# mpotse/ParMmg

Hardware: AMD Instinct MI355X
Metric: new-mesh points located+interpolated/sec (Mpts/s) and HBM GB/s, 1/2/4/8 GPU (higher is better)
Workload: dtype f64

## Files before the change

parmmg_amd/csrc/pmmg_hip.hip:

```cpp
#include <hip/hip_ext.h>
#include <hip/hip_runtime.h>

#include <math.h>
#include <stdarg.h>
#include <stdint.h>
#include <stdio.h>
#include <stdlib.h>
#include <string.h>

#include <algorithm>
#include <chrono>
#include <condition_variable>
#include <functional>
#include <mutex>
#include <string>
#include <thread>
#include <type_traits>
#include <vector>

#include "pmmg_device.hpp"
#include "pmmg_prep.hpp"
#include "pmmg_sort.hpp"
#include "pmmg_vol.hpp"
#include "pmmg_bdy.hpp"
#include "pmmg_fallback.hpp"
#include "pmmg_snapshot.hpp"
#include "pmmg_quality.hpp"
#include "pmmg_meshstats.hpp"
#include "pmmg_graph.hpp"
#include "pmmg_comm.hpp"

using namespace pmmg;

namespace {


typedef void (*VolFn)(Bg, const Frame *, const unsigned long long *, int, const double *, const uint8_t *,
                      const int *, int, DevStats *, Slots, int *, int8_t *, int, const int *, int, ContArgs, MapArgs);

struct LayoutEntry {
  int c[6];
  VolFn fn;
  VolFn fn_packed;
  VolFn fn_packed2;
  VolFn map_fn, map_fn_packed, map_fn_packed2;
};

template <int NP, int A, int B, int C, int D, int E, int F, int MAP = 0>
constexpr VolFn packed_fn() {
  using L = PackedLayout<A, B, C, D, E, F>;
  if constexpr (L::valid() && L::passes_ok(NP)) return k_vol<NP, A, B, C, D, E, F, MAP>;
  else return nullptr;
}
#define PMMG_LAYOUT(a, b, c, d, e, f)                                                                    \
  {{a, b, c, d, e, f}, k_vol<0, a, b, c, d, e, f>, packed_fn<1, a, b, c, d, e, f>(),                    \
   packed_fn<2, a, b, c, d, e, f>(), k_vol<0, a, b, c, d, e, f, 1>, packed_fn<1, a, b, c, d, e, f, 1>(), \
   packed_fn<2, a, b, c, d, e, f, 1>()}
const LayoutEntry kLayouts[] = {
    PMMG_LAYOUT(6, 1, 3, 6, 0, 0), PMMG_LAYOUT(6, 1, 3, 6, 1, 0), PMMG_LAYOUT(1, 1, 0, 0, 0, 0),
    PMMG_LAYOUT(1, 1, 1, 1, 1, 1), PMMG_LAYOUT(1, 1, 1, 0, 0, 0), PMMG_LAYOUT(6, 0, 0, 0, 0, 0),
    PMMG_LAYOUT(1, 0, 0, 0, 0, 0), PMMG_LAYOUT(6, 1, 0, 0, 0, 0), PMMG_LAYOUT(1, 1, 3, 6, 0, 0),
    PMMG_LAYOUT(0, 0, 0, 0, 0, 0),
};
#undef PMMG_LAYOUT

VolFn pick_layout(const Slots &S, int passes = 0, bool map = false) {
  for (const LayoutEntry &e : kLayouts) {
    int n = 0;
    while (n < 6 && e.c[n] > 0) n++;
    if (n != S.n) continue;
    bool ok = true;
    for (int j = 0; j < n; j++) ok = ok && (S.s[j].code == e.c[j]);
    if (!ok) continue;
    if (!S.rec) return map ? e.map_fn : e.fn;
    if (passes == 0) {
      int k = 0;
      for (int j = 0; j < n; j++) k += e.c[j];
      passes = k > 8 ? 2 : 1;
    }
    const VolFn p1 = map ? e.map_fn_packed : e.fn_packed, p2 = map ? e.map_fn_packed2 : e.fn_packed2;
    const VolFn a = passes == 2 ? p2 : p1, b = passes == 2 ? p1 : p2;
    return a ? a : b;
  }
  if (S.rec) return nullptr;
  return map ? k_vol<0, -1, 0, 0, 0, 0, 0, 1> : k_vol<0, -1, 0, 0, 0, 0, 0>;
}

bool packed_supported(int met_size, int nfield, const int *fsize) {
  Slots S{};
  S.rec = reinterpret_cast<const double *>(16);
  if (met_size) S.s[S.n++].code = met_size;
  for (int j = 0; j < nfield && S.n < kMaxSlot; j++) S.s[S.n++].code = fsize[j];
  return pick_layout(S) != nullptr;
}

}


struct CtxBufs {
  DevBuf o_xyz, o_tetv, o_adja, o_triv, o_adjt, o_met, o_rec;
  std::vector<DevBuf> o_f;
  DevBuf o_tet4;
  DevBuf frame, stats, grid, sgrid, order_v, order_b, xq;
  DevBuf cohd;
  DevBuf axh;
  DevBuf bkeys, bkeys2, bvals, bvals2;
  DevBuf rs_hist, rs_csum;
  DevBuf cls_cnt;
  DevBuf oflag;
  DevBuf qmin;
  DevBuf fb_vol, fb_bdy, best, nac, cres, bbest, bnac, bcres;
  DevBuf fbp_vol, fbp_bdy;
  DevBuf fbg_vol_c, fbg_vol_u, fbg_vol_i, fbg_bdy_c, fbg_bdy_u, fbg_bdy_i;
  DevBuf h_xyz, h_cls, h_met, h_elem, h_hit;
  std::vector<DevBuf> h_f;
  SnapCache snap_cache;
  StatsCache stats_cache;
  GraphCache graph_cache;
  struct Kept {
    DevBuf xyz, met;
    std::vector<DevBuf> f;
    int np = 0, met_size = 0;
    std::vector<int> fsize;
    bool valid = false;
  };
  std::vector<Kept> kept;
  DevBuf carry_dsrc, carry_need, carry_ids, carry_cnt, carry_rows, carry_bc;
  DevBuf map_own;
  DevBuf map_need;
  DevBuf start_tab;
  DevBuf ag_send, ag_recv, ag_off, ag_chk;
};

enum {
  EV_START, EV_FRAME, EV_PREP, EV_ORDER, EV_VOL0, EV_WALK, EV_JOIN, EV_END, EV_BDY0, EV_BDY1, EV_RESET,
  EV_SB0, EV_ORDER2, EV_FILL, EV_COUNT
};

struct pmmg_hip_ctx : CtxBufs {
  int device = 0;
  int options = 0;
  hipStream_t stream = nullptr;
  hipStream_t stream2 = nullptr;
  hipStream_t stream3 = nullptr;
  hipStream_t stream_f = nullptr;
  char err[512] = {0};
  Bg bg{};
  int met_size = 0;
  int nfield = 0;
  std::vector<int> fsize;
  std::vector<const double *> fin;
  const double *met = nullptr;
  const double *rec = nullptr;
  int rstride = 0;
  void *grid_clean_p = nullptr, *sgrid_clean_p = nullptr;
  long long grid_clean_n = 0, sgrid_clean_n = 0;
  hipEvent_t ev[EV_COUNT] = {};
  bool pending = false;
  void *stage[2] = {nullptr, nullptr};
  void *stage_dev[2] = {nullptr, nullptr};
  hipEvent_t stage_ev[2] = {};
  int stage_i = 0;
  struct Pool *pool = nullptr;
  int edge_hash = 1;
  hipStream_t cstream = nullptr;
  std::thread snap;
  int snap_ok = 1;
  int verbose = 0;
  int tpc = 8;
  int pack_passes = 0;
  int ev_vol0 = EV_VOL0;
  int *flag_host = nullptr;
  int *flag_host_dev = nullptr;
  int srf_g = 0;
  int srf_mult = 8;
  int bin_bits = kBinBitsCoherent;
  int maxstep = 1024;
  int fanmax = kFanMax;
  int last_host_np = 0, last_host_met = 0;
  std::vector<int> last_host_fsize;
  int carry_slot = -1, carry_np = 0;
  bool carry_bg = false;
  std::vector<int> carry_src;
  int64_t bytes_up = 0;
  const int *map_src = nullptr;
  int map_np = 0;
  bool start_valid = false;
  std::vector<pmmg_hip_ctx *> lanes;
  bool borrowed_streams = false;
  ncclComm_t comm = nullptr;
  bool comm_owned = false;
  int comm_rank = 0, comm_size = 0;
  int group_lanes = 3;
  struct Pool *lane_pool = nullptr;
  int filter_steps = 64;
};

static void set_err(pmmg_hip_ctx *c, const char *fmt, ...) {
  if (!c) return;
  va_list ap;
  va_start(ap, fmt);
  vsnprintf(c->err, sizeof(c->err), fmt, ap);
  va_end(ap);
  fprintf(stderr, "[parmmg_hip] %s\n", c->err);
}

#define HIPCK(ctx, expr)                                                                             \
  do {                                                                                               \
    hipError_t e_ = (expr);                                                                          \
    if (e_ != hipSuccess) {                                                                          \
      set_err((ctx), "%s failed: %s (%s:%d)", #expr, hipGetErrorString(e_), __FILE__, __LINE__);   \
      return 0;                                                                                      \
    }                                                                                                \
  } while (0)

static hipError_t ctx_d2h(pmmg_hip_ctx *c, void *dst, const void *src, size_t n) {
  hipError_t e = hipMemcpyAsync(dst, src, n, hipMemcpyDeviceToHost, c->stream);
  return e != hipSuccess ? e : hipStreamSynchronize(c->stream);
}

static int ensure(pmmg_hip_ctx *c, DevBuf &b, size_t bytes) {
  const hipError_t e = b.ensure(bytes);
  if (e != hipSuccess) {
    set_err(c, "hipMalloc(&b.p, bytes) failed: %s (%s:%d)", hipGetErrorString(e), __FILE__, __LINE__);
    return 0;
  }
  return 1;
}

static int copy_stream(pmmg_hip_ctx *c) {
  if (!c->cstream) HIPCK(c, hipStreamCreateWithFlags(&c->cstream, hipStreamNonBlocking));
  return 1;
}


struct Pool {
  std::vector<std::thread> th;
  std::mutex mu;
  std::condition_variable cv, done;
  std::function<void(size_t, size_t)> fn;
  size_t n = 0, parts = 0, next = 0, left = 0;
  unsigned long long gen = 0;
  bool stop = false;
  explicit Pool(int nthreads) {
    for (int t = 0; t < nthreads; t++) th.emplace_back([this] { loop(); });
  }
  ~Pool() {
    {
      std::lock_guard<std::mutex> g(mu);
      stop = true;
    }
    cv.notify_all();
    for (auto &t : th) t.join();
  }
  bool take(size_t &b, size_t &e) {
    if (next >= parts) return false;
    const size_t p = next++;
    b = n * p / parts;
    e = n * (p + 1) / parts;
    return true;
  }
  void loop() {
    unsigned long long seen = 0;
    std::unique_lock<std::mutex> lk(mu);
    for (;;) {
      cv.wait(lk, [&] { return stop || gen != seen; });
      if (stop) return;
      seen = gen;
      size_t b, e;
      while (take(b, e)) {
        lk.unlock();
        fn(b, e);
        lk.lock();
        if (--left == 0) done.notify_all();
      }
    }
  }
  void run(size_t count, size_t nparts, std::function<void(size_t, size_t)> f) {
    if (nparts <= 1 || th.empty()) {
      f(0, count);
      return;
    }
    std::unique_lock<std::mutex> lk(mu);
    fn = std::move(f);
    n = count;
    parts = nparts;
    next = 0;
    left = nparts;
    gen++;
    cv.notify_all();
    size_t b, e;
    while (take(b, e)) {
      lk.unlock();
      fn(b, e);
      lk.lock();
      left--;
    }
    done.wait(lk, [&] { return left == 0; });
  }
};

static int env_int(const char *name, int def);

constexpr size_t kStageBytes = 32u << 20;
constexpr size_t kStageMin = 4u << 20;
constexpr unsigned long long kSentinel = 0x7FF4A5A5A5A5A5A5ULL;

__global__ __launch_bounds__(kBlock) void k_copy16(const ntd2 *src, ntd2 *dst, long long n) {
  for (long long j = blockIdx.x * (long long)blockDim.x + threadIdx.x; j < n; j += (long long)gridDim.x * blockDim.x)
    __builtin_nontemporal_store(__builtin_nontemporal_load(src + j), dst + j);
}
__global__ __launch_bounds__(kBlock) void k_copy1(const char *src, char *dst, long long n) {
  for (long long j = blockIdx.x * (long long)blockDim.x + threadIdx.x; j < n; j += (long long)gridDim.x * blockDim.x)
    dst[j] = src[j];
}

static int stage_ready(pmmg_hip_ctx *c) {
  if (c->stage[0]) return 1;
  for (int b = 0; b < 2; b++) {
    HIPCK(c, hipHostMalloc(&c->stage[b], kStageBytes, hipHostMallocDefault));
    HIPCK(c, hipHostGetDevicePointer(&c->stage_dev[b], c->stage[b], 0));
    HIPCK(c, hipEventCreateWithFlags(&c->stage_ev[b], hipEventDisableTiming));
  }
  if (!c->pool) {
    const int hw = (int)std::thread::hardware_concurrency();
    c->pool = new Pool(env_int("PMMG_HIP_HOST_THREADS", hw > 16 ? 16 : (hw > 1 ? hw : 1)) - 1);
  }
  return 1;
}

static void par_copy(pmmg_hip_ctx *c, void *dst, const void *src, size_t n) {
  const size_t parts = n >= (8u << 20) ? c->pool->th.size() + 1 : 1;
  c->pool->run(n, parts, [&](size_t b, size_t e) { memcpy((char *)dst + b, (const char *)src + b, e - b); });
}

static int h2d(pmmg_hip_ctx *c, void *dst, const void *src, size_t bytes, hipStream_t s) {
  if (bytes == 0) return 1;
  c->bytes_up += (int64_t)bytes;
  if (bytes < kStageMin) {
    HIPCK(c, hipMemcpyAsync(dst, src, bytes, hipMemcpyHostToDevice, s));
    return 1;
  }
  if (!stage_ready(c)) return 0;
  for (size_t off = 0; off < bytes;) {
    const int b = c->stage_i;
    c->stage_i ^= 1;
    const size_t n = bytes - off < kStageBytes ? bytes - off : kStageBytes;
    HIPCK(c, hipEventSynchronize(c->stage_ev[b]));
    par_copy(c, c->stage[b], (const char *)src + off, n);
    HIPCK(c, hipMemcpyAsync((char *)dst + off, c->stage[b], n, hipMemcpyHostToDevice, s));
    HIPCK(c, hipEventRecord(c->stage_ev[b], s));
    off += n;
  }
  return 1;
}

struct AllRows {
  bool operator()(size_t, const char *) const { return true; }
};
static double now_s() {
  return std::chrono::duration<double>(std::chrono::steady_clock::now().time_since_epoch()).count();
}

template <class Keep>
static int d2h_rows(pmmg_hip_ctx *c, void *dst, const void *src, size_t nrows, size_t row, const Keep &keep) {
  const size_t bytes = nrows * row;
  if (bytes == 0) return 1;
  if (!stage_ready(c)) return 0;
  double t_wait = 0.0;
  const double t_start = now_s();
  const size_t per = kStageBytes / row;
  const size_t nch = (nrows + per - 1) / per;
  auto issue = [&](size_t j) -> int {
    const int b = (int)(j & 1);
    const size_t r0 = j * per, n = (nrows - r0 < per ? nrows - r0 : per) * row;
    const char *from = (const char *)src + r0 * row;
    if (((uintptr_t)from & 15) == 0 && (n & 15) == 0) {
      hipLaunchKernelGGL(k_copy16, dim3(1024), dim3(kBlock), 0, c->stream, (const ntd2 *)from, (ntd2 *)c->stage_dev[b],
                         (long long)(n / 16));
    } else {
      hipLaunchKernelGGL(k_copy1, dim3(1024), dim3(kBlock), 0, c->stream, from, (char *)c->stage_dev[b], (long long)n);
    }
    HIPCK(c, hipGetLastError());
    HIPCK(c, hipEventRecord(c->stage_ev[b], c->stream));
    return 1;
  };
  if (!issue(0)) return 0;
  for (size_t j = 0; j < nch; j++) {
    const int b = (int)(j & 1);
    const double t0 = now_s();
    HIPCK(c, hipEventSynchronize(c->stage_ev[b]));
    const double t1 = now_s();
    t_wait += t1 - t0;
    if (j + 1 < nch && !issue(j + 1)) return 0;
    const size_t r0 = j * per, nr = nrows - r0 < per ? nrows - r0 : per;
    const char *sb = (const char *)c->stage[b];
    char *db = (char *)dst + r0 * row;
    if constexpr (std::is_same<Keep, AllRows>::value) {
      par_copy(c, db, sb, nr * row);
    } else {
      c->pool->run(nr, nr >= 65536 ? c->pool->th.size() + 1 : 1, [&](size_t a, size_t e) {
        size_t r = a;
        while (r < e) {
          while (r < e && !keep(r0 + r, sb + r * row)) r++;
          const size_t s0 = r;
          while (r < e && keep(r0 + r, sb + r * row)) r++;
          if (r > s0) memcpy(db + s0 * row, sb + s0 * row, (r - s0) * row);
        }
      });
    }
  }
  if (c->verbose)
    fprintf(stderr, "[parmmg_hip] d2h %zu rows x %zu B: %.2f ms DMA wait, %.2f ms in total\n", nrows, row,
            1e3 * t_wait, 1e3 * (now_s() - t_start));
  return 1;
}

static int upload(pmmg_hip_ctx *c, DevBuf &b, const void *src, size_t bytes, hipStream_t s = nullptr) {
  if (!ensure(c, b, bytes)) return 0;
  return h2d(c, b.p, src, bytes, s ? s : c->stream);
}

static void invalidate_bg(pmmg_hip_ctx *c) {
  c->bg.ne = c->bg.nt = c->bg.np = 0;
  c->bg.tetv = c->bg.adja = nullptr;
  c->bg.triv = c->bg.adjt = nullptr;
  c->bg.xyz = nullptr;
  c->start_valid = false;
}

static int snap_join(pmmg_hip_ctx *c) {
  if (c->snap.joinable()) c->snap.join();
  if (!c->snap_ok) {
    c->snap_ok = 1;
    invalidate_bg(c);
    return 0;
  }
  return 1;
}
// ... 537 lines not shown
    set_err(c, "set_solutions_packed: a carry-over is armed; it takes pmmg_hip_set_solutions (the kept rows are "
               "per-solution arrays)");
    carry_disarm(c);
    return 0;
  }
  c->met_size = met_size;
  c->nfield = nfield;
  c->fsize.assign(field_size, field_size + nfield);
  c->fin.assign(nfield, nullptr);
  c->met = nullptr;
  c->rstride = (K + 1) & ~1;
  if (where == PMMG_HIP_DEVICE) {
    c->rec = rec;
    return 1;
  }
  if (!copy_stream(c) || !upload(c, c->o_rec, rec, sizeof(double) * c->rstride * np, c->cstream)) return 0;
  c->rec = (const double *)c->o_rec.p;
  HIPCK(c, hipStreamSynchronize(c->cstream));
  return 1;
}

constexpr int kSmallGroup = 1 << 20;

static int grid_dim(long long n, int per_cell, int gmax) {
  double g = cbrt((double)n / (double)per_cell);
  int gi = (int)g;
  if (gi < 1) gi = 1;
  if (gi > gmax) gi = gmax;
  return gi;
}

static int blocks_for(long long n, int cap) {
  long long b = (n + kBlock - 1) / kBlock;
  if (b < 1) b = 1;
  if (b > cap) b = cap;
  return (int)b;
}

static void launch_vol_fallbacks(pmmg_hip_ctx *c, const Slots &S, const double *xyz_new, int *elem_out,
                                 int8_t *hit_out, hipEvent_t stop = nullptr) {
  const Bg &bg = c->bg;
  hipStream_t s = c->stream;
  DevStats *st = (DevStats *)c->stats.p;
  const int *fb = (const int *)c->fb_vol.p;
  const int gv = (int)std::min<long long>(kFbGridVol, std::max<long long>(64, bg.ne / 16384)) & ~7;
  hipLaunchKernelGGL(k_vol_exhaust_accept, dim3(gv), dim3(kBlock), 0, s, bg, xyz_new, fb, st,
                     (int *)c->best.p, (int *)c->nac.p, (const int *)c->fbg_vol_c.p, (const int *)c->fbg_vol_i.p, S,
                     elem_out, hit_out);
  hipExtLaunchKernelGGL(k_vol_exhaust_closest, dim3(gv), dim3(kBlock), 0, s, nullptr, stop, 0, bg, xyz_new, fb, st,
                        (const int *)c->nac.p, (FbPart *)c->fbp_vol.p, (int *)c->cres.p, S, elem_out, hit_out);
}

static void launch_bdy_fallbacks(pmmg_hip_ctx *c, hipStream_t s, const Slots &S, const double *xyz_new,
                                 int *elem_out, int8_t *hit_out, hipEvent_t stop = nullptr) {
  const Bg &bg = c->bg;
  DevStats *st = (DevStats *)c->stats.p;
  const int *fb = (const int *)c->fb_bdy.p;
  const int gb = (int)std::min<long long>(kFbGridBdy, std::max<long long>(32, bg.nt / 4096)) & ~7;
  hipLaunchKernelGGL(k_bdy_exhaust_accept, dim3(gb), dim3(kBlock), 0, s, bg, xyz_new, fb, st,
                     (int *)c->bbest.p, (int *)c->bnac.p, (const int *)c->fbg_bdy_c.p, (const int *)c->fbg_bdy_i.p, S,
                     elem_out, hit_out);
  hipExtLaunchKernelGGL(k_bdy_exhaust_closest, dim3(gb), dim3(kBlock), 0, s, nullptr, stop, 0, bg, xyz_new, fb, st,
                        (const int *)c->bnac.p, (FbPart *)c->fbp_bdy.p, (int *)c->bcres.p, S, elem_out, hit_out);
}

static int start_tables(pmmg_hip_ctx *c) {
  if (c->start_valid) return 1;
  const Bg &bg = c->bg;
  const size_t n = 2 * (size_t)bg.np;
  if (!ensure(c, c->start_tab, sizeof(int) * n)) return 0;
  unsigned *tab = (unsigned *)c->start_tab.p;
  HIPCK(c, hipMemsetAsync(tab, 0xFF, sizeof(int) * n, c->stream));
  hipLaunchKernelGGL(k_start_tet, dim3(blocks_for(bg.ne, 16384)), dim3(kBlock), 0, c->stream, bg, tab);
  if (bg.nt > 0)
    hipLaunchKernelGGL(k_start_tri, dim3(blocks_for(bg.nt, 4096)), dim3(kBlock), 0, c->stream, bg, tab + bg.np);
  hipLaunchKernelGGL(k_start_fin, dim3(blocks_for((long long)n, 4096)), dim3(kBlock), 0, c->stream, tab, (long long)n);
  HIPCK(c, hipGetLastError());
  c->start_valid = true;
  return 1;
}


constexpr int kSeedLanes = 4;
constexpr int kBboxStride = 64;
constexpr int kHistStride = 256;
constexpr int kBdyBpx = 512;
constexpr int kXcdRun = 64;

struct Call {
  pmmg_hip_ctx *c;
  int np_new;
  const double *xyz_new;
  const uint8_t *pclass;
  int *elem_out;
  int8_t *hit_out;
  Bg bg;
  hipStream_t s, sb, sc;
  Slots S;
  VolFn vol_fn;
  MapArgs ma;
  int *need;
  int force;
  int g, gs;
  long long ng, nsg, ncls;
  Frame *fr;
  DevStats *st;
  unsigned long long *grid, *sgrid;
  int *order_v, *order_b;
  const int *flag;
};

static int call_slots(Call &k, double *met_out, double *const *fields_out, double *rec_out, const int *map_src) {
  pmmg_hip_ctx *c = k.c;
  Slots &S = k.S;
  S.n = 0;
  S.has_met = c->met_size ? 1 : 0;
  if (rec_out && !c->rec) {
    set_err(c, "locate_interp_rec: output records need packed input records (pmmg_hip_set_solutions_packed)");
    return 0;
  }
  if (c->met_size) {
    if (!met_out && !rec_out) {
      set_err(c, "locate_interp: met_out is NULL");
      return 0;
    }
    S.s[S.n++] = Slot{c->met, met_out, c->met_size, c->met_size, c->met_size};
  }
  for (int j = 0; j < c->nfield; j++) {
    if (!rec_out && (!fields_out || !fields_out[j])) {
      set_err(c, "locate_interp: fields_out[%d] is NULL", j);
      return 0;
    }
    S.s[S.n++] = Slot{c->fin[j], rec_out ? nullptr : fields_out[j], c->fsize[j], c->fsize[j], c->fsize[j]};
  }
  if (c->rec) {
    S.rec = c->rec;
    int off = 0;
    for (int j = 0; j < S.n; j++) {
      S.s[j].in = c->rec + off;
      S.s[j].istride = c->rstride;
      if (rec_out) {
        S.s[j].out = rec_out + off;
        S.s[j].ostride = c->rstride;
      }
      off += S.s[j].code;
    }
    S.rec_out = rec_out;
  }
  k.vol_fn = pick_layout(S, c->pack_passes, map_src != nullptr);
  if (!k.vol_fn) {
    set_err(c, "locate_interp: no packed-record kernel for this slot layout");
    return 0;
  }
  k.ma = MapArgs{nullptr, nullptr, nullptr};
  k.need = nullptr;
  if (map_src) {
    if (!start_tables(c) || !ensure(c, c->map_need, 2 * sizeof(int))) return 0;
    k.need = (int *)c->map_need.p;
    k.ma = MapArgs{map_src, (const int *)c->start_tab.p, (const int *)c->start_tab.p + k.bg.np};
  }
  return 1;
}

static int call_scratch(Call &k) {
  pmmg_hip_ctx *c = k.c;
  Bg &bg = k.bg;
  k.g = grid_dim(bg.ne, c->tpc, 1024);
  k.gs = bg.nt <= 0 ? 1 : (c->srf_g > 0 ? c->srf_g : grid_dim((long long)bg.nt * c->srf_mult, 2, 1024));
  const size_t nq = (size_t)k.np_new;
  k.ng = (long long)k.g * k.g * k.g;
  k.nsg = bg.nt > 0 ? (long long)k.gs * k.gs * k.gs : 0;
  k.ncls = (long long)(nq / kScanChunk + 1);
  if (!ensure(c, c->frame, sizeof(Frame)) || !ensure(c, c->stats, sizeof(DevStats) + kStatParts * sizeof(StatPart)) ||
      !ensure(c, c->grid, 8 * (size_t)k.ng) || !ensure(c, c->sgrid, 8 * (size_t)k.nsg) ||
      !ensure(c, c->order_v, 4 * nq) || !ensure(c, c->order_b, 4 * nq) || !ensure(c, c->bkeys, 4 * nq) ||
      !ensure(c, c->bkeys2, 4 * nq) || !ensure(c, c->bvals, 4 * nq) || !ensure(c, c->cls_cnt, 4 * (size_t)k.ncls) ||
      !ensure(c, c->fb_vol, 4 * nq) || !ensure(c, c->fb_bdy, 4 * nq) || !ensure(c, c->best, 4 * nq) ||
      !ensure(c, c->nac, 4 * nq) || !ensure(c, c->cres, 4 * nq) || !ensure(c, c->bbest, 4 * nq) ||
      !ensure(c, c->bnac, 4 * nq) || !ensure(c, c->bcres, 4 * nq) ||
      !ensure(c, c->fbp_vol, sizeof(FbPart) * (size_t)kFbPartCap) ||
      !ensure(c, c->fbp_bdy, sizeof(FbPart) * 256 * (size_t)kFbGridBdy) ||
      !ensure(c, c->fbg_vol_c, 4 * (size_t)(kFbCells + 1)) || !ensure(c, c->fbg_vol_u, 4 * (size_t)kFbCells) ||
      !ensure(c, c->fbg_vol_i, 4 * nq) || !ensure(c, c->fbg_bdy_c, 4 * (size_t)(kFbCells + 1)) ||
      !ensure(c, c->fbg_bdy_u, 4 * (size_t)kFbCells) || !ensure(c, c->fbg_bdy_i, 4 * nq))
    return 0;
  if (!ensure(c, c->xq, sizeof(int) * kXqStride * (size_t)bg.np) || !ensure(c, c->oflag, 2 * sizeof(int)) ||
      !ensure(c, c->cohd, sizeof(double) * kCohSamples) ||
      !ensure(c, c->axh, sizeof(int) * 3 * kMapBins * (size_t)kHistBlocks))
    return 0;
  bg.xq = (const int *)c->xq.p;
  k.fr = (Frame *)c->frame.p;
  k.st = (DevStats *)c->stats.p;
  k.grid = (unsigned long long *)c->grid.p;
  k.sgrid = (unsigned long long *)c->sgrid.p;
  k.order_v = (int *)c->order_v.p;
  k.order_b = (int *)c->order_b.p;
  k.flag = (const int *)c->oflag.p;
  k.force = (c->options & PMMG_HIP_OPT_SORT) ? 1 : (c->options & PMMG_HIP_OPT_NOSORT) ? 0 : -1;
  if (k.force < 0 && k.np_new < kSmallGroup) k.force = 0;
  if (k.force < 0 && !c->flag_host) {
    void *p = nullptr;
    HIPCK(c, hipHostMalloc(&p, 64, hipHostMallocCoherent | hipHostMallocMapped));
    c->flag_host = (int *)p;
    void *d = nullptr;
    HIPCK(c, hipHostGetDevicePointer(&d, p, 0));
    c->flag_host_dev = (int *)d;
  }
  if (k.force < 0) c->flag_host[0] = -1;
  return 1;
}

static int launch_frame_seeds(Call &k) {
  pmmg_hip_ctx *c = k.c;
  const Bg &bg = k.bg;
  const int force = k.force;
  hipStream_t s = k.s;
  const long long ng_clr = (c->grid.p == c->grid_clean_p && k.ng <= c->grid_clean_n) ? 0 : k.ng;
  const long long nsg_clr = (c->sgrid.p == c->sgrid_clean_p && k.nsg <= c->sgrid_clean_n) ? 0 : k.nsg;
  c->grid_clean_n = c->sgrid_clean_n = 0;
  hipExtLaunchKernelGGL(k_reset, dim3(blocks_for(ng_clr > nsg_clr ? ng_clr : nsg_clr, 2048)), dim3(kBlock), 0, s,
                        c->ev[EV_START], force >= 0 ? c->ev[EV_RESET] : nullptr, 0, k.fr, k.st, k.grid, ng_clr, k.sgrid,
                        nsg_clr, (int *)c->oflag.p, force, c->bin_bits);
  if (k.need) {
    HIPCK(c, hipMemsetAsync(k.need, 0, 2 * sizeof(int), s));
    hipLaunchKernelGGL(k_map_count, dim3(blocks_for(k.np_new, 2048)), dim3(kBlock), 0, s, k.pclass,
                       (long long)k.np_new, k.ma, bg.np, bg.ne, bg.nt, k.need);
  }
  hipExtLaunchKernelGGL(k_bbox, dim3(std::max(force < 0 ? kCohBlocks : 1, blocks_for(bg.np / kBboxStride + 1, 256))),
                        dim3(kBlock), 0, s, nullptr, c->ev[EV_FRAME], 0, (const double *)bg.xyz, bg.np, k.fr,
                        kBboxStride, k.g, k.gs, 1 << kBinBitsAxis, k.xyz_new, k.np_new,
                        force < 0 ? (int *)c->oflag.p : nullptr, (double *)c->cohd.p,
                        force < 0 ? c->flag_host_dev : nullptr);
  hipLaunchKernelGGL(k_quantize, dim3(std::max(kHistBlocks, blocks_for(3LL * bg.np, 8192))), dim3(kBlock), 0, s,
                     bg.xyz, (long long)bg.np, (const Frame *)k.fr, (int *)c->xq.p, kHistStride, (int *)c->axh.p);
  hipLaunchKernelGGL(k_axis_map, dim3(3), dim3(kBlock), 0, s, (const int *)c->axh.p, k.fr, k.g);
  HIPCK(c, hipGetLastError());

  HIPCK(c, hipStreamWaitEvent(k.sb, c->ev[force < 0 ? EV_FRAME : EV_RESET], 0));
  if (force == 1 || bg.nt <= 0) HIPCK(c, hipEventRecord(c->ev[EV_SB0], k.sb));
  k.sc = k.sb;
  if (force != 0) {
    if (!c->stream3 && hipStreamCreateWithFlags(&c->stream3, hipStreamNonBlocking) != hipSuccess)
      c->stream3 = nullptr;
    if (c->stream3) k.sc = c->stream3;
    HIPCK(c, hipStreamWaitEvent(k.sc, c->ev[EV_FRAME], 0));
  }
  HIPCK(c, hipGetLastError());

  const long long nsamp = k.ng < bg.ne ? k.ng : bg.ne;
  hipExtLaunchKernelGGL(k_seed_vol, dim3((blocks_for((nsamp + kSeedBatch - 1) / kSeedBatch, 8192) + 7) & ~7),
                        dim3(kBlock), 0, s, nullptr, c->ev[EV_PREP], 0, bg, k.fr, k.grid, k.g, nsamp, kSeedLanes,
                        (const int *)k.need);
  HIPCK(c, hipGetLastError());
  return 1;
}

static bool launch_cls(Call &k, bool order_end) {
  pmmg_hip_ctx *c = k.c;
  if (k.force == 1 || k.bg.nt <= 0) return false;
  int *bc = (int *)c->cls_cnt.p;
  hipExtLaunchKernelGGL(k_cls_count, dim3((unsigned)k.ncls), dim3(kBlock), 0, k.sb, c->ev[EV_SB0], nullptr, 0,
                        k.pclass, (long long)k.np_new, (int)PMMG_PT_BDY, bc, k.flag, 0);
  hipLaunchKernelGGL(k_scan_top, dim3(1), dim3(kBlock), 0, k.sb, bc, (int)k.ncls, &k.st->nbdy, k.flag, 0);
  hipExtLaunchKernelGGL(k_cls_scatter, dim3((unsigned)k.ncls), dim3(kBlock), 0, k.sb, nullptr,
                        order_end ? c->ev[EV_ORDER] : nullptr, 0, k.pclass, (long long)k.np_new, (int)PMMG_PT_BDY,
                        (const int *)bc, k.order_b, k.flag, 0);
  return order_end;
}

static int launch_morton(Call &k) {
  pmmg_hip_ctx *c = k.c;
  const int np_new = k.np_new;
  if (k.force == 0 || np_new <= 0) return 1;
  hipStream_t sc = k.sc;
  const size_t nq = (size_t)np_new;
  const int ntile = (int)((np_new + kRsTile - 1) / kRsTile);
  const long long nh = 256LL * ntile;
  const int nch = (int)((nh + kScanChunk - 1) / kScanChunk);
  if (!ensure(c, c->bvals2, 4 * nq) || !ensure(c, c->rs_hist, 4 * (size_t)nh) || !ensure(c, c->rs_csum, 4 * (size_t)nch))
    return 0;
  unsigned *k0 = (unsigned *)c->bkeys.p, *k1 = (unsigned *)c->bkeys2.p;
  int *v0 = (int *)c->bvals.p, *v1 = (int *)c->bvals2.p, *hist = (int *)c->rs_hist.p, *csum = (int *)c->rs_csum.p;
  const int tgrid = std::min(ntile, kRsGrid);
  hipLaunchKernelGGL(k_bin_keys, dim3(tgrid), dim3(kBlock), 0, sc, k.xyz_new, k.pclass, np_new, (const Frame *)k.fr,
                     k.flag, k0, v0, k.st, kRsTile, ntile, hist);
  for (int pass = 0; pass < 3; pass++) {
    const unsigned *kin = pass == 1 ? k1 : k0;
    const int *vin = pass == 1 ? v1 : v0;
    unsigned *kout = pass == 1 ? k0 : k1;
    int *vout = pass == 1 ? v0 : (pass == 0 ? v1 : k.order_v);
    if (pass > 0)
      hipLaunchKernelGGL(k_rs_hist, dim3(tgrid), dim3(kBlock), 0, sc, kin, np_new, 8 * pass, ntile, hist, k.flag, 1);
    hipLaunchKernelGGL(k_rs_scan_local, dim3(nch), dim3(kBlock), 0, sc, hist, (int)nh, csum, k.flag, 1);
    hipLaunchKernelGGL(k_scan_top, dim3(1), dim3(kBlock), 0, sc, csum, nch, (int *)nullptr, k.flag, 1);
    hipLaunchKernelGGL(k_rs_scan_add, dim3(nch), dim3(kBlock), 0, sc, hist, (int)nh, (const int *)csum, k.flag, 1);
    hipLaunchKernelGGL(k_rs_scatter, dim3(tgrid), dim3(kBlock), 0, sc, kin, vin, np_new, 8 * pass, ntile,
                       (const int *)hist, kout, vout, k.flag, 1);
  }
  hipLaunchKernelGGL(k_bin_split, dim3(blocks_for(np_new, 4096)), dim3(kBlock), 0, sc, (const int *)k.order_v,
                     k.order_b, (const DevStats *)k.st, k.flag);
  return 1;
}

static int srf_head(Call &k) {
  pmmg_hip_ctx *c = k.c;
  const Bg &bg = k.bg;
  if (k.np_new >= kSmallGroup) HIPCK(c, hipStreamWaitEvent(k.sb, c->ev[EV_PREP], 0));
  if (bg.nt <= 0) HIPCK(c, hipEventRecord(c->ev[EV_BDY0], k.sb));
  if (bg.nt > 0) {
    if (k.force == 0) HIPCK(c, hipStreamWaitEvent(k.sb, c->ev[EV_FRAME], 0));
    hipExtLaunchKernelGGL(k_seed_srf, dim3(blocks_for(bg.nt, 4096)), dim3(kBlock), 0, k.sb, c->ev[EV_BDY0], nullptr,
                          0, bg, (const Frame *)k.fr, k.sgrid, k.gs,
                          k.need ? (const int *)k.need + 1 : (const int *)nullptr);
  }
  return 1;
}

static void launch_bdy(Call &k) {
  pmmg_hip_ctx *c = k.c;
  const auto bdy_fn = k.ma.src ? k_bdy<1> : k_bdy<0>;
  hipLaunchKernelGGL(bdy_fn, dim3(8 * blocks_for((k.np_new + 7) / 8, kBdyBpx)), dim3(kBlock), 0,
                     k.sb, k.bg, (const Frame *)k.fr, (const unsigned long long *)k.sgrid, k.gs, k.xyz_new,
                     (const int *)k.order_b, k.S, k.elem_out, k.hit_out, (int *)c->fb_bdy.p, k.st, c->maxstep,
                     FbInit{(int *)c->bbest.p},
                     FbGridBufs{(int *)c->fbg_bdy_c.p, (int *)c->fbg_bdy_u.p, (int *)c->fbg_bdy_i.p}, k.ma);
}

static int srf_tail(Call &k) {
  pmmg_hip_ctx *c = k.c;
  bool rec = false;
  const bool fill = k.nsg >= kRefillCells;
  if (k.bg.nt > 0) {
    hipLaunchKernelGGL(k_fb_grid, dim3(1), dim3(kBlock), 0, k.sb, k.xyz_new, (const int *)c->fb_bdy.p, k.st, 1,
                       FbGridBufs{(int *)c->fbg_bdy_c.p, (int *)c->fbg_bdy_u.p, (int *)c->fbg_bdy_i.p});
    launch_bdy_fallbacks(c, k.sb, k.S, k.xyz_new, k.elem_out, k.hit_out, fill ? nullptr : c->ev[EV_BDY1]);
    rec = !fill;
    HIPCK(c, hipGetLastError());
    if (fill) {
      hipExtLaunchKernelGGL(k_fill64, dim3(blocks_for((k.nsg + 1) / 2, 2048)), dim3(kBlock), 0, k.sb, nullptr,
                            c->ev[EV_BDY1], 0, k.sgrid, k.nsg, ~0ULL);
      rec = true;
      c->sgrid_clean_p = c->sgrid.p;
      c->sgrid_clean_n = k.nsg;
    }
  }
  if (!rec) HIPCK(c, hipEventRecord(c->ev[EV_BDY1], k.sb));
  return 1;
}

static int launch_vol(Call &k) {
  pmmg_hip_ctx *c = k.c;
  if (k.force != 0 && k.sc != k.sb) HIPCK(c, hipStreamWaitEvent(k.s, c->ev[EV_ORDER2], 0));
  c->ev_vol0 = k.force == 0 ? EV_PREP : EV_VOL0;
  if (c->ev_vol0 == EV_VOL0) HIPCK(c, hipEventRecord(c->ev[EV_VOL0], k.s));
  const ContArgs ca{(int *)c->fb_vol.p, FbInit{(int *)c->best.p}, c->maxstep};
  hipExtLaunchKernelGGL(k.vol_fn, dim3((k.np_new + 63) / 64), dim3(64), 0, k.s, nullptr, c->ev[EV_WALK], 0, k.bg,
                        (const Frame *)k.fr, (const unsigned long long *)k.grid, k.g, k.xyz_new, k.pclass,
                        (const int *)k.order_v, k.np_new, k.st, k.S, k.elem_out, k.hit_out, c->filter_steps, k.flag,
                        kXcdRun, ca, k.ma);
  return 1;
}

static int launch_tail(Call &k) {
  pmmg_hip_ctx *c = k.c;
  hipStream_t s = k.s;
  const bool refill = k.ng >= kRefillCells;
  if (refill) {
    if (!c->stream_f) HIPCK(c, hipStreamCreateWithFlags(&c->stream_f, hipStreamNonBlocking));
    HIPCK(c, hipStreamWaitEvent(c->stream_f, c->ev[EV_WALK], 0));
    hipExtLaunchKernelGGL(k_fill64, dim3(blocks_for((k.ng + 1) / 2, 2048)), dim3(kBlock), 0, c->stream_f, nullptr,
                          c->ev[EV_FILL], 0, k.grid, k.ng, ~0ULL);
    HIPCK(c, hipGetLastError());
    c->grid_clean_p = c->grid.p;
    c->grid_clean_n = k.ng;
  }
  HIPCK(c, hipGetLastError());
  hipLaunchKernelGGL(k_fb_grid, dim3(1), dim3(kBlock), 0, s, k.xyz_new, (const int *)c->fb_vol.p, k.st, 0,
                     FbGridBufs{(int *)c->fbg_vol_c.p, (int *)c->fbg_vol_u.p, (int *)c->fbg_vol_i.p});
  launch_vol_fallbacks(c, k.S, k.xyz_new, k.elem_out, k.hit_out, c->ev[EV_JOIN]);
  HIPCK(c, hipGetLastError());
  HIPCK(c, hipStreamWaitEvent(s, c->ev[EV_BDY1], 0));
  if (refill) HIPCK(c, hipStreamWaitEvent(s, c->ev[EV_FILL], 0));
  HIPCK(c, hipEventRecord(c->ev[EV_END], s));
  c->pending = true;
  return 1;
}

static int run_device(pmmg_hip_ctx *c, int np_new, const double *xyz_new, const uint8_t *pclass, double *met_out,
                      double *const *fields_out, int *elem_out, int8_t *hit_out, double *rec_out = nullptr,
                      const int *map_src = nullptr) {
  Call k{};
  k.c = c;
  k.np_new = np_new;
  k.xyz_new = xyz_new;
  k.pclass = pclass;
  k.elem_out = elem_out;
  k.hit_out = hit_out;
  k.bg = c->bg;
  k.s = c->stream;
  k.sb = k.sc = c->stream2;
  if (!call_slots(k, met_out, fields_out, rec_out, map_src) || !call_scratch(k) || !launch_frame_seeds(k)) return 0;
  const bool pre = k.force < 0;
  bool ord = false;
  if (pre) {
    if (!launch_cls(k, true)) HIPCK(c, hipEventRecord(c->ev[EV_ORDER], k.sb));
    ord = true;
    if (!srf_head(k)) return 0;
    HIPCK(c, hipGetLastError());
    HIPCK(c, hipEventSynchronize(c->ev[EV_FRAME]));
    const int f = __atomic_load_n(&c->flag_host[0], __ATOMIC_ACQUIRE);
    if (f != 0 && f != 1) {
      set_err(c, "locate_interp: the query order decision did not arrive (%d)", f);
      return 0;
    }
    k.force = f;
  } else {
    ord = launch_cls(k, k.force == 0);
  }
  if (!launch_morton(k)) return 0;
  HIPCK(c, hipGetLastError());
  if (!ord) HIPCK(c, hipEventRecord(c->ev[EV_ORDER], k.sb));
  if (k.force != 0) HIPCK(c, hipEventRecord(c->ev[EV_ORDER2], k.sc));
  if (pre && !launch_vol(k)) return 0;
  if (k.sc != k.sb && k.force != 0) HIPCK(c, hipStreamWaitEvent(k.sb, c->ev[EV_ORDER2], 0));
  if (!pre && !srf_head(k)) return 0;
  if (k.bg.nt > 0) launch_bdy(k);
  if (!srf_tail(k)) return 0;
  if (!pre && !launch_vol(k)) return 0;
  HIPCK(c, hipGetLastError());
  return launch_tail(k);
}

static int collect_stats(pmmg_hip_ctx *c, pmmg_hip_stats *out) {
  DevStats h;
  int order[2] = {0, 0};
  HIPCK(c, ctx_d2h(c, order, c->oflag.p, sizeof(order)));
  std::vector<StatPart> parts(kStatParts);
  HIPCK(c, ctx_d2h(c, &h, c->stats.p, sizeof(DevStats)));
  HIPCK(c, ctx_d2h(c, parts.data(), (const DevStats *)c->stats.p + 1, kStatParts * sizeof(StatPart)));
  unsigned long long cnt[kNumCnt] = {0}, steps = 0, stepmax = 0;
  for (const StatPart &pt : parts) {
    for (int j = 0; j < kNumCnt; j++) cnt[j] += pt.cnt[j];
    steps += pt.steps;
    if (pt.stepmax > stepmax) stepmax = pt.stepmax;
  }
  memset(out, 0, sizeof(*out));
  out->nvol = order[0] == 1 ? (int64_t)h.nvol : (int64_t)cnt[kCntVolQueries];
  out->nbdy = h.nbdy;
  out->nvol_walk = (int64_t)cnt[PMMG_HIT_VOL_WALK];
  out->nvol_exhaust = (int64_t)cnt[PMMG_HIT_VOL_EXHAUST];
  out->nvol_closest = (int64_t)cnt[PMMG_HIT_VOL_CLOSEST];
  out->nvol_exact = (int64_t)cnt[kCntExact];
  out->nbdy_face = (int64_t)cnt[PMMG_HIT_BDY_FACE];
  out->nbdy_edge = (int64_t)cnt[PMMG_HIT_BDY_EDGE];
  out->nbdy_vertex = (int64_t)cnt[PMMG_HIT_BDY_VERTEX];
  out->nbdy_wedge = (int64_t)cnt[PMMG_HIT_BDY_WEDGE];
  out->nbdy_cone = (int64_t)cnt[PMMG_HIT_BDY_CONE];
  out->nbdy_exhaust = (int64_t)cnt[PMMG_HIT_BDY_EXHAUST];
  out->nbdy_stale = (int64_t)cnt[PMMG_HIT_BDY_STALE];
  out->nbdy_closest = (int64_t)cnt[PMMG_HIT_BDY_CLOSEST];
  out->steps_total = (int64_t)steps;
  out->stepmax = (int64_t)stepmax;
  out->wave_iters = (int64_t)cnt[kCntWaveIters];
  out->sorted = order[0] == 1;
  out->nvol_noseed = (int64_t)cnt[kCntNoSeed];
  out->nvol_stuck = (int64_t)cnt[kCntStuck];
  out->nvol_limit = (int64_t)cnt[kCntLimit];
  {
    int ad = 0;
    HIPCK(c, ctx_d2h(c, &ad, &((const Frame *)c->frame.p)->adaptive, sizeof(int)));
    out->seed_map_axes = ad;
    out->nbdy_fanscan = (int64_t)cnt[kCntFanScan];
    out->nvol_src = (int64_t)cnt[kCntVolSrc];
    out->nbdy_src = (int64_t)cnt[kCntBdySrc];
  }
  float ms = 0.f;
  HIPCK(c, hipEventElapsedTime(&ms, c->ev[EV_START], c->ev[EV_PREP]));
  out->ms_prepare = ms;
  HIPCK(c, hipEventElapsedTime(&ms, c->ev[EV_SB0], c->ev[EV_ORDER]));
  out->ms_sort = ms;
  HIPCK(c, hipEventElapsedTime(&ms, c->ev[c->ev_vol0], c->ev[EV_WALK]));
  out->ms_vol = out->ms_vol_locate = ms;
  HIPCK(c, hipEventElapsedTime(&ms, c->ev[EV_BDY0], c->ev[EV_BDY1]));
  out->ms_bdy = ms;
  HIPCK(c, hipEventElapsedTime(&ms, c->ev[EV_WALK], c->ev[EV_JOIN]));
  out->ms_fallback = ms;
  HIPCK(c, hipEventElapsedTime(&ms, c->ev[EV_START], c->ev[EV_END]));
  out->ms_total = ms;
  return 1;
}

int pmmg_hip_sync(pmmg_hip_ctx *c, pmmg_hip_stats *stats) {
  if (!enter(c)) return 0;
  for (pmmg_hip_ctx *l : c->lanes)
    if (hipStreamSynchronize(l->stream) != hipSuccess) {
      set_err(c, "sync: group lane failed: %s", l->err);
      return 0;
    }
  HIPCK(c, hipStreamSynchronize(c->stream));
  if (stats && c->pending) return collect_stats(c, stats);
  return 1;
}

static int take_point_map(pmmg_hip_ctx *c, int np_new, const int **src) {
  *src = c->map_src;
  c->map_src = nullptr;
  if (*src && c->map_np != np_new) {
    set_err(c, "locate_interp: the point map was armed for %d new points, the call has %d", c->map_np, np_new);
    return 0;
  }
  return 1;
}

int pmmg_hip_set_point_map(pmmg_hip_ctx *c, int np_new, const int *src, int where) {
  if (!c) return 0;
  c->map_src = nullptr;
  if (np_new <= 0 || !src) {
    set_err(c, "set_point_map: np_new = %d or src NULL", np_new);
    return 0;
  }
  if (where == PMMG_HIP_DEVICE) {
    c->map_src = src;
  } else {
    HIPCK(c, hipSetDevice(c->device));
    if (!snap_join(c)) return 0;
    if (!upload(c, c->map_own, src, sizeof(int) * (size_t)np_new)) return 0;
    c->map_src = (const int *)c->map_own.p;
  }
  c->map_np = np_new;
  return 1;
}

int pmmg_hip_start_elements(pmmg_hip_ctx *c, int *start_tet, int *start_tri, int where) {
  if (!enter(c)) return 0;
  if (c->bg.ne <= 0) {
    set_err(c, "start_elements: no background set");
    return 0;
  }
  if (!start_tables(c)) return 0;
  const size_t bytes = sizeof(int) * (size_t)c->bg.np;
  const int *tab = (const int *)c->start_tab.p;
  const hipMemcpyKind kind = where == PMMG_HIP_DEVICE ? hipMemcpyDeviceToDevice : hipMemcpyDeviceToHost;
  if (start_tet) HIPCK(c, hipMemcpyAsync(start_tet, tab, bytes, kind, c->stream));
  if (start_tri) HIPCK(c, hipMemcpyAsync(start_tri, tab + c->bg.np, bytes, kind, c->stream));
  HIPCK(c, hipStreamSynchronize(c->stream));
  return 1;
}

int pmmg_hip_locate_interp(pmmg_hip_ctx *c, int np_new, const double *xyz_new, const uint8_t *pclass,
                           double *met_out, double *const *fields_out, int *elem_out, int8_t *hit_out,
                           pmmg_hip_stats *stats, int where) {
  if (!c) return 0;
  const int *map_src = nullptr;
  if (!take_point_map(c, np_new, &map_src)) return 0;
  HIPCK(c, hipSetDevice(c->device));
  if (!snap_join(c)) return 0;
  if (c->bg.ne <= 0) {
    set_err(c, "locate_interp: no background set");
    return 0;
  }
  if (np_new <= 0) {
    if (stats) memset(stats, 0, sizeof(*stats));
    return 1;
  }
  if (!xyz_new || !pclass) {
    set_err(c, "locate_interp: xyz_new / pclass is NULL");
    return 0;
  }
  if (where == PMMG_HIP_DEVICE) {
    if (((uintptr_t)met_out & 15) && c->met_size == 6) {
      set_err(c, "locate_interp: a device tensor output must be 16-byte aligned");
      return 0;
    }
    if (!run_device(c, np_new, xyz_new, pclass, met_out, fields_out, elem_out, hit_out, nullptr, map_src)) return 0;
    if (stats) return pmmg_hip_sync(c, stats);
    return 1;
  }
  size_t n = (size_t)np_new;
  const double t0 = now_s();
  if (!upload(c, c->h_xyz, xyz_new, sizeof(double) * 3 * n)) return 0;
  if (!upload(c, c->h_cls, pclass, n)) return 0;
  double *dmet = nullptr;
  auto sentinel_fill = [&](DevBuf &b, size_t ndbl) -> int {
    if (!ensure(c, b, sizeof(double) * ndbl)) return 0;
    hipLaunchKernelGGL(k_fill64, dim3(blocks_for((long long)ndbl, 4096)), dim3(kBlock), 0, c->stream,
                       (unsigned long long *)b.p, (long long)ndbl, kSentinel);
    return 1;
  };
  if (c->met_size) {
    if (!met_out) {
      set_err(c, "locate_interp: met_out is NULL");
      return 0;
    }
    if (!sentinel_fill(c->h_met, (size_t)c->met_size * n)) return 0;
    dmet = (double *)c->h_met.p;
  }
  c->h_f.resize(c->nfield);
  std::vector<double *> dfields(c->nfield > 0 ? c->nfield : 1, nullptr);
  for (int j = 0; j < c->nfield; j++) {
    if (!fields_out || !fields_out[j]) {
      set_err(c, "locate_interp: fields_out[%d] is NULL", j);
      return 0;
    }
    if (!sentinel_fill(c->h_f[j], (size_t)c->fsize[j] * n)) return 0;
    dfields[j] = (double *)c->h_f[j].p;
  }
  if (!ensure(c, c->h_elem, sizeof(int) * n) || !ensure(c, c->h_hit, n)) return 0;
  HIPCK(c, hipMemsetAsync(c->h_hit.p, 0, n, c->stream));
  if (!run_device(c, np_new, (const double *)c->h_xyz.p, (const uint8_t *)c->h_cls.p, dmet, dfields.data(),
                  (int *)c->h_elem.p, (int8_t *)c->h_hit.p, nullptr, map_src))
    return 0;
  const double t1 = now_s();
  std::vector<int8_t> hh(n);
  if (!d2h_rows(c, hh.data(), c->h_hit.p, n, 1, AllRows{})) return 0;
  const double t2 = now_s();
  auto written = [&](size_t, const char *row) {
    unsigned long long u;
    memcpy(&u, row, 8);
    return u != kSentinel;
  };
  auto processed = [&](size_t r, const char *) { return hh[r] != 0; };
  if (dmet && !d2h_rows(c, met_out, dmet, n, sizeof(double) * c->met_size, written)) return 0;
  for (int j = 0; j < c->nfield; j++)
    if (!d2h_rows(c, fields_out[j], dfields[j], n, sizeof(double) * c->fsize[j], written)) return 0;
  if (elem_out && !d2h_rows(c, elem_out, c->h_elem.p, n, sizeof(int), processed)) return 0;
  if (hit_out)
    c->pool->run(n, n >= 65536 ? c->pool->th.size() + 1 : 1, [&](size_t a, size_t e) {
      for (size_t r = a; r < e; r++)
        if (hh[r]) hit_out[r] = hh[r];
    });
  if (c->verbose)
    fprintf(stderr, "[parmmg_hip] host locate: uploads + enqueue %.2f ms, step + hit codes %.2f ms, rows %.2f ms\n",
            1e3 * (t1 - t0), 1e3 * (t2 - t1), 1e3 * (now_s() - t2));
  c->last_host_np = np_new;
  c->last_host_met = c->met_size;
  c->last_host_fsize = c->fsize;
  if (stats) return collect_stats(c, stats);
  return 1;
}

int pmmg_hip_locate_interp_rec(pmmg_hip_ctx *c, int np_new, const double *xyz_new, const uint8_t *pclass,
                               double *rec_out, int *elem_out, int8_t *hit_out, pmmg_hip_stats *stats, int where) {
  if (!c) return 0;
  const int *map_src = nullptr;
  if (!take_point_map(c, np_new, &map_src)) return 0;
  HIPCK(c, hipSetDevice(c->device));
  if (!snap_join(c)) return 0;
  if (where != PMMG_HIP_DEVICE) {
    set_err(c, "locate_interp_rec: device pointers only (PMMG_HIP_DEVICE)");
    return 0;
  }
  if (c->bg.ne <= 0) {
    set_err(c, "locate_interp_rec: no background set");
    return 0;
  }
  if (!c->rec) {
    set_err(c, "locate_interp_rec: output records need packed input records (pmmg_hip_set_solutions_packed)");
    return 0;
  }
  if (np_new <= 0) {
    if (stats) memset(stats, 0, sizeof(*stats));
    return 1;
  }
  if (!xyz_new || !pclass || !rec_out || ((uintptr_t)rec_out & 15)) {
    set_err(c, "locate_interp_rec: xyz_new / pclass / rec_out NULL or rec_out not 16-byte aligned");
    return 0;
  }
  if (!run_device(c, np_new, xyz_new, pclass, nullptr, nullptr, elem_out, hit_out, rec_out, map_src)) return 0;
  if (stats) return pmmg_hip_sync(c, stats);
  return 1;
}


int pmmg_hip_keep(pmmg_hip_ctx *c, int slot) {
  if (!c) return 0;
  if (slot < 0 || slot >= 1024) {
    set_err(c, "keep: slot %d out of [0, 1024)", slot);
    return 0;
  }
  if (c->last_host_np <= 0) {
    set_err(c, "keep: no host-mode pmmg_hip_locate_interp to keep since the last keep");
    return 0;
  }
  if ((int)c->kept.size() <= slot) c->kept.resize(slot + 1);
  pmmg_hip_ctx::Kept &k = c->kept[slot];
// ... 581 lines not shown
```

Baseline: 5513.

## Overlap surface-grid refill on fill stream and shrink seed_srf block size

Moves the surface-grid reset (k_fill64 on sgrid) off the boundary stream's tail onto the separate fill stream. It is triggered by a new event recorded right after the boundary walk kernel, so the reset can overlap with the boundary fallbacks and the volume tail. The end event now also waits on the new fill event. Separately, the surface seed kernel is launched with 64-thread blocks and proportionally more blocks. This adds cross-stream dependencies, and the fill could race if the fallbacks still read sgrid after the walk kernel.

```diff
diff --git a/parmmg_amd/csrc/pmmg_hip.hip b/parmmg_amd/csrc/pmmg_hip.hip
--- a/parmmg_amd/csrc/pmmg_hip.hip
+++ b/parmmg_amd/csrc/pmmg_hip.hip
@@ -134,7 +134,7 @@
 
 enum {
   EV_START, EV_FRAME, EV_PREP, EV_ORDER, EV_VOL0, EV_WALK, EV_JOIN, EV_END, EV_BDY0, EV_BDY1, EV_RESET,
-  EV_SB0, EV_ORDER2, EV_FILL, EV_COUNT
+  EV_SB0, EV_ORDER2, EV_FILL, EV_BDYK, EV_FILLS, EV_COUNT
 };
 
 struct pmmg_hip_ctx : CtxBufs {
@@ -1278,6 +1278,8 @@
   return 1;
 }
 
+static bool srf_refill(const Call &k) { return k.bg.nt > 0 && k.nsg >= kRefillCells; }
+
 static int srf_head(Call &k) {
   pmmg_hip_ctx *c = k.c;
   const Bg &bg = k.bg;
@@ -1285,8 +1287,8 @@
   if (bg.nt <= 0) HIPCK(c, hipEventRecord(c->ev[EV_BDY0], k.sb));
   if (bg.nt > 0) {
     if (k.force == 0) HIPCK(c, hipStreamWaitEvent(k.sb, c->ev[EV_FRAME], 0));
-    hipExtLaunchKernelGGL(k_seed_srf, dim3(blocks_for(bg.nt, 4096)), dim3(kBlock), 0, k.sb, c->ev[EV_BDY0], nullptr,
-                          0, bg, (const Frame *)k.fr, k.sgrid, k.gs,
+    hipExtLaunchKernelGGL(k_seed_srf, dim3((kBlock / 64) * blocks_for(bg.nt, 4096)), dim3(64), 0, k.sb,
+                          c->ev[EV_BDY0], nullptr, 0, bg, (const Frame *)k.fr, k.sgrid, k.gs,
                           k.need ? (const int *)k.need + 1 : (const int *)nullptr);
   }
   return 1;
@@ -1295,30 +1297,22 @@
 static void launch_bdy(Call &k) {
   pmmg_hip_ctx *c = k.c;
   const auto bdy_fn = k.ma.src ? k_bdy<1> : k_bdy<0>;
-  hipLaunchKernelGGL(bdy_fn, dim3(8 * blocks_for((k.np_new + 7) / 8, kBdyBpx)), dim3(kBlock), 0,
-                     k.sb, k.bg, (const Frame *)k.fr, (const unsigned long long *)k.sgrid, k.gs, k.xyz_new,
-                     (const int *)k.order_b, k.S, k.elem_out, k.hit_out, (int *)c->fb_bdy.p, k.st, c->maxstep,
-                     FbInit{(int *)c->bbest.p},
-                     FbGridBufs{(int *)c->fbg_bdy_c.p, (int *)c->fbg_bdy_u.p, (int *)c->fbg_bdy_i.p}, k.ma);
+  hipExtLaunchKernelGGL(bdy_fn, dim3(8 * blocks_for((k.np_new + 7) / 8, kBdyBpx)), dim3(kBlock), 0, k.sb, nullptr,
+                        srf_refill(k) ? c->ev[EV_BDYK] : nullptr, 0, k.bg, (const Frame *)k.fr,
+                        (const unsigned long long *)k.sgrid, k.gs, k.xyz_new, (const int *)k.order_b, k.S, k.elem_out,
+                        k.hit_out, (int *)c->fb_bdy.p, k.st, c->maxstep, FbInit{(int *)c->bbest.p},
+                        FbGridBufs{(int *)c->fbg_bdy_c.p, (int *)c->fbg_bdy_u.p, (int *)c->fbg_bdy_i.p}, k.ma);
 }
 
 static int srf_tail(Call &k) {
   pmmg_hip_ctx *c = k.c;
   bool rec = false;
-  const bool fill = k.nsg >= kRefillCells;
   if (k.bg.nt > 0) {
     hipLaunchKernelGGL(k_fb_grid, dim3(1), dim3(kBlock), 0, k.sb, k.xyz_new, (const int *)c->fb_bdy.p, k.st, 1,
                        FbGridBufs{(int *)c->fbg_bdy_c.p, (int *)c->fbg_bdy_u.p, (int *)c->fbg_bdy_i.p});
-    launch_bdy_fallbacks(c, k.sb, k.S, k.xyz_new, k.elem_out, k.hit_out, fill ? nullptr : c->ev[EV_BDY1]);
-    rec = !fill;
+    launch_bdy_fallbacks(c, k.sb, k.S, k.xyz_new, k.elem_out, k.hit_out, c->ev[EV_BDY1]);
+    rec = true;
     HIPCK(c, hipGetLastError());
-    if (fill) {
-      hipExtLaunchKernelGGL(k_fill64, dim3(blocks_for((k.nsg + 1) / 2, 2048)), dim3(kBlock), 0, k.sb, nullptr,
-                            c->ev[EV_BDY1], 0, k.sgrid, k.nsg, ~0ULL);
-      rec = true;
-      c->sgrid_clean_p = c->sgrid.p;
-      c->sgrid_clean_n = k.nsg;
-    }
   }
   if (!rec) HIPCK(c, hipEventRecord(c->ev[EV_BDY1], k.sb));
   return 1;
@@ -1340,15 +1334,24 @@
 static int launch_tail(Call &k) {
   pmmg_hip_ctx *c = k.c;
   hipStream_t s = k.s;
-  const bool refill = k.ng >= kRefillCells;
+  const bool refill = k.ng >= kRefillCells, srefill = srf_refill(k);
+  if ((refill || srefill) && !c->stream_f)
+    HIPCK(c, hipStreamCreateWithFlags(&c->stream_f, hipStreamNonBlocking));
   if (refill) {
-    if (!c->stream_f) HIPCK(c, hipStreamCreateWithFlags(&c->stream_f, hipStreamNonBlocking));
     HIPCK(c, hipStreamWaitEvent(c->stream_f, c->ev[EV_WALK], 0));
     hipExtLaunchKernelGGL(k_fill64, dim3(blocks_for((k.ng + 1) / 2, 2048)), dim3(kBlock), 0, c->stream_f, nullptr,
                           c->ev[EV_FILL], 0, k.grid, k.ng, ~0ULL);
     HIPCK(c, hipGetLastError());
     c->grid_clean_p = c->grid.p;
     c->grid_clean_n = k.ng;
+  }
+  if (srefill) {
+    HIPCK(c, hipStreamWaitEvent(c->stream_f, c->ev[EV_BDYK], 0));
+    hipExtLaunchKernelGGL(k_fill64, dim3(blocks_for((k.nsg + 1) / 2, 2048)), dim3(kBlock), 0, c->stream_f, nullptr,
+                          c->ev[EV_FILLS], 0, k.sgrid, k.nsg, ~0ULL);
+    HIPCK(c, hipGetLastError());
+    c->sgrid_clean_p = c->sgrid.p;
+    c->sgrid_clean_n = k.nsg;
   }
   HIPCK(c, hipGetLastError());
   hipLaunchKernelGGL(k_fb_grid, dim3(1), dim3(kBlock), 0, s, k.xyz_new, (const int *)c->fb_vol.p, k.st, 0,
@@ -1357,6 +1360,7 @@
   HIPCK(c, hipGetLastError());
   HIPCK(c, hipStreamWaitEvent(s, c->ev[EV_BDY1], 0));
   if (refill) HIPCK(c, hipStreamWaitEvent(s, c->ev[EV_FILL], 0));
+  if (srefill) HIPCK(c, hipStreamWaitEvent(s, c->ev[EV_FILLS], 0));
   HIPCK(c, hipEventRecord(c->ev[EV_END], s));
   c->pending = true;
   return 1;
```

Measured after the change: 5492. No clear change (-0.4%).
